# alphacep/vosk-tts

Hardware: AMD Instinct MI355X
Metric: audio_samples_per_sec (higher is better)
Workload: dtype f32

## Files before the change

### include/vits_mi355_debug.h

```cpp
#ifndef VITS_MI355_DEBUG_H
#define VITS_MI355_DEBUG_H
#include "vits_mi355.h"
#ifdef __cplusplus
extern "C" {
#endif

void vits_debug_force_tile(int mode);
void vits_debug_attention_impl(int impl);
void vits_debug_fast_path(int on);
void vits_debug_ks_waves(int nw);
void vits_debug_ln_stats(int on);
void vits_debug_persist(int mask);
void vits_debug_persist_spin(int limit);
void vits_debug_persist_when(int max_others_in_flight);
void vits_debug_persist_rearm_ms(int ms);
int vits_debug_persist_runs(vits_model* m);
void vits_debug_wn_fold(int on);
void vits_debug_conv_wp(int mode);
int vits_debug_decoder_needs(const vits_hparams* hp, int32_t* out, int32_t cap);
void vits_debug_conv_sp(int mode);
void vits_debug_no_bf16x3(int on);
void vits_debug_tail_impl(int impl);
void vits_debug_poison_workspace(int on);
int vits_debug_plain_attention(int device, const float* qkv, const int64_t* lengths, int32_t B, int32_t C, int32_t T,
                               int32_t n_heads, float* out);

int vits_debug_clock_probe(int device, int32_t duration_us, double* ghz, int32_t n);

#ifdef __cplusplus
}
#endif
#endif
```

### vosk_tts_amd/csrc/conv_small.hip.h

```cpp
#pragma once
#include "conv_mfma.hip.h"

#define C16_MAXU 20

template <typename F>
static void pack_conv_weights16(float* dst, int Mpad16, int Cin, int K, F src) {
  const int n_u = Cin / CONV_CI_T * K;
  for (int mb = 0; mb < Mpad16 / 16; ++mb)
    for (int u = 0; u < n_u; ++u)
      for (int lane = 0; lane < 64; ++lane)
        for (int q = 0; q < 4; ++q) {
          const int chunk = u / K, kk = u % K;
          const int ci = chunk * CONV_CI_T + 4 * q + (lane >> 4);
          const int row = mb * 16 + (lane & 15);
          dst[(((size_t)mb * n_u + u) * 64 + lane) * 4 + q] = src(row, ci, kk);
        }
}

static inline int c16_row_pitch(int row) { return row <= 16 ? 16 : (row <= 48 ? 48 : 80); }

#define DDS_MAXI 16
#define DDS_XP 36
__device__ __forceinline__ float c16_gelu(float v) { return 0.5f * v * (1.0f + erff(v * 0.70710678118654752440f)); }
template <int NG, int NC>
// ... 710 lines not shown
    return;
  }
  const bool masked = P.out_mask && ecol >= len_raw;
#pragma unroll
  for (int i = 0; i < NE; ++i) {
    float r = sum[i] + ebias[i];
    if (masked) r = 0.f;
    r += eres[i];
    if (eok[i]) {
      G.y[eoff[i]] = r;
      if (G.y2) G.y2[eoff[i]] = r;
    }
  }
  CONV_DBG(5);
}

template <int NW>
__global__ void __launch_bounds__(NW * 64, 4) conv_wp_kernel(const ConvParams P) {
  extern __shared__ float lds[];
  kernarg_warm<sizeof(ConvParams)>();
  const int tid = threadIdx.x, lane = tid & 63;
  const int wave = __builtin_amdgcn_readfirstlane(tid >> 6);
  CONV_DBG(0);
  int mt, grp, nt, b;
  if (!conv_decode_block(P, mt, grp, nt, b)) return;
  const ConvGroup& G = P.g[grp];
  switch (G.K) {
    case 3: conv_wp_body<NW, 3>(P, G, lds, mt, nt, b, wave, lane); break;
    case 7: conv_wp_body<NW, 7>(P, G, lds, mt, nt, b, wave, lane); break;
    case 11: conv_wp_body<NW, 11>(P, G, lds, mt, nt, b, wave, lane); break;
    default: conv_wp_body<NW, 0>(P, G, lds, mt, nt, b, wave, lane); break;
  }
}
```

### vosk_tts_amd/csrc/engine.hip

```cpp
#include <hip/hip_runtime.h>

#include <math.h>
#include <stdarg.h>
#include <stdio.h>
#include <stdlib.h>
#include <string.h>
#include <fcntl.h>
#include <sys/file.h>
#include <unistd.h>

#include <algorithm>
#include <atomic>
#include <chrono>
#include <map>
#include <mutex>
#include <string>
#include <tuple>
#include <vector>

#include "../../include/vits_mi355.h"
#include "../../include/vits_mi355_debug.h"
#include "conv_mfma.hip.h"
#include "conv_small.hip.h"
#include "conv_sp.hip.h"
#include "conv_bf3.hip.h"
#include "kernels_misc.hip.h"
#include "persist.hip.h"

static thread_local char g_err[512];
static int fail(int code, const char* fmt, ...) {
  va_list ap;
  va_start(ap, fmt);
  vsnprintf(g_err, sizeof g_err, fmt, ap);
  va_end(ap);
  return code;
}
#define HIP_TRY(expr)                                                                              \
  do {                                                                                             \
    hipError_t e_ = (expr);                                                                        \
    if (e_ != hipSuccess) return fail(VITS_ERR_DEVICE, "%s failed: %s (%s:%d)", #expr, hipGetErrorString(e_), __FILE__, __LINE__); \
  } while (0)
#define TRY(expr)              \
  do {                         \
    int rc_ = (expr);          \
// ... 467 lines not shown
  const long long until = g_ps_off_until_ns.load(), now = steady_ns();
  out->active_mask = (until && now < until) ? 0 : g_persist.load();
  out->off_for_ms = (until && now < until) ? (int32_t)((until - now + 999999) / 1000000) : 0;
  out->timeouts = g_ps_timeouts.load();
  out->rearms = g_ps_rearms.load();
  out->launches = -1;
  out->process_owns_device = -1;
  if (m) {
    out->launches = vits_debug_persist_runs(m);
    std::lock_guard<std::mutex> g(g_tok_mu);
    if (m->device >= 0 && m->device < 64) out->process_owns_device = g_proc_lock[m->device];
  }
  return VITS_OK;
}
void vits_debug_persist_spin(int limit) {
  const int lim = limit > 0 ? limit : 0;
  g_ps_spin_limit = lim;
  std::lock_guard<std::mutex> g(g_models_mu);
  for (vits_model* m : g_models) {
    hipSetDevice(m->device);
    hipDeviceSynchronize();
    hipMemcpy(m->ps_dbg, &lim, sizeof(int), hipMemcpyHostToDevice);
  }
}
int vits_debug_persist_runs(vits_model* m) {
  if (!m) return -1;
  int v[2] = {0, 0};
  hipSetDevice(m->device);
  hipDeviceSynchronize();
  if (hipMemcpy(v, m->ps_dbg, sizeof v, hipMemcpyDeviceToHost) != hipSuccess) return -1;
  return v[1];
}
void vits_debug_conv_wp(int mode) { g_wp_mode = mode; }
int vits_debug_decoder_needs(const vits_hparams* hp, int32_t* out, int32_t cap) {
  if (!hp || !out || hp->n_ups < 0 || hp->n_ups > VITS_MAX_UPS || hp->n_resd < 0 || hp->n_resd > VITS_MAX_RESD || hp->n_resk < 0 || hp->n_resk > VITS_MAX_RESK)
    return -fail(VITS_ERR_ARG, "decoder_needs: bad arguments");
  for (int i = 0; i < hp->n_ups; ++i) if (hp->up_rates[i] < 1) return -fail(VITS_ERR_ARG, "decoder_needs: bad up_rates");
  if (hp->dec_type < 0 || hp->dec_type > 3) return -fail(VITS_ERR_ARG, "decoder_needs: dec_type %d unsupported", hp->dec_type);
  if ((hp->dec_type == 0 || hp->dec_type == 2 || hp->dec_type == 3) && (hp->istft_hop < 1 || hp->subbands < 1 || hp->istft_n_fft < 1))
    return -fail(VITS_ERR_ARG, "decoder_needs: bad tail geometry");
  if ((hp->dec_type == 0 || hp->dec_type == 2) && hp->pqmf_taps < 0) return -fail(VITS_ERR_ARG, "decoder_needs: bad synthesis filter length");
  if (hp->dec_type == 3 && hp->subbands != 1) return -fail(VITS_ERR_ARG, "decoder_needs: single-band decoder with subbands != 1");
  const DecNeeds N = decoder_needs(*hp, true);
  std::vector<int32_t> v = {N.pre_out + 3, N.pre_out, N.post_out, N.tail_cols};
  for (int i = 0; i < hp->n_ups; ++i) {
    v.push_back(N.ups_q[i]);
    for (int d = 0; d < hp->n_resd; ++d) v.push_back(N.c1_out[i][d]);
    for (int d = 0; d < hp->n_resd; ++d) v.push_back(N.c2_out[i][d]);
  }
  for (int i = 0; i < (int)v.size() && i < cap; ++i) out[i] = v[i];
  return (int)v.size();
}
void vits_debug_conv_sp(int mode) { g_sp_mode = mode; }
int vits_debug_clock_probe(int device, int32_t duration_us, double* ghz, int32_t n) {
  if (!ghz || n < 1 || n > 1024 || duration_us < 1 || duration_us > 2000000 || device < 0 || device >= 64) return fail(VITS_ERR_ARG, "clock probe: bad arguments");
  HIP_TRY(hipSetDevice(device));
  static std::mutex mu;
  static hipStream_t st[64];
  static double* buf[64];
  std::lock_guard<std::mutex> g(mu);
  if (!st[device]) {
    HIP_TRY(hipStreamCreateWithFlags(&st[device], hipStreamNonBlocking));
    if (hipMalloc((void**)&buf[device], sizeof(double) * 1024) != hipSuccess) { buf[device] = nullptr; return fail(VITS_ERR_NOMEM, "clock probe: device alloc failed"); }
  }
  if (!buf[device]) return fail(VITS_ERR_NOMEM, "clock probe: no buffer");
  hipLaunchKernelGGL(clock_probe_kernel, dim3(n), dim3(64), 0, st[device], buf[device], (long long)duration_us * 100);
// ... 166 lines not shown
```

### vosk_tts_amd/csrc/engine_launch.hip.h

```cpp
#pragma once
struct ProfScope {
  vits_session* s; bool on;
  ProfScope(vits_session* s_, const char* name, double flops, const char* kernel = "-") : s(s_), on(s_->profile) {
    if (!on) return;
    ProfRec r; r.name = name; r.kernel = kernel; r.flops = flops;
    hipEventCreate(&r.e0); hipEventCreate(&r.e1);
    hipEventRecord(r.e0, s->stream);
    s->prof.push_back(r);
  }
  void set_kernel(const char* k) { if (on) s->prof.back().kernel = k; }
  void add_template_arg(int v) {
    if (!on) return;
    std::string& k = s->prof.back().kernel;
    if (!k.empty() && k.back() == '>') { k.pop_back(); k += "," + std::to_string(v) + ">"; }
  }
  ~ProfScope() { if (on) hipEventRecord(s->prof.back().e1, s->stream); }
};


static bool big_lds_needed(std::atomic<unsigned long long>& done);
static void persist_launch(vits_session* s, vits_session::PersistProg& pp, const char* name, const float* d_noise = nullptr, float nsw = 0.f,
                           uint64_t seed = 0, const int64_t* d_ids = nullptr, const int* d_forced = nullptr, float length_scale = 1.f,
                           float noise_scale = 0.f) {
  vits_model* m = s->m;
// ... 224 lines not shown
static thread_local int g_no_bf3 = 0;
static bool conv_wp_ok(const ConvParams& P, int epi, int halo, bool small) {
  static const int env_mode = getenv("VITS_CONV_WP") ? atoi(getenv("VITS_CONV_WP")) : 0;
  const int mode = g_wp_mode ? g_wp_mode : env_mode;
  if (mode == 1 || epi != EPI_STORE) return false;
  if (P.x_ch_sign != 1 || P.x_ch_off || P.tile_start || P.ups_u || P.reflect || P.in_scale != 1.f || P.ln_g || P.dds_y2 || P.ln_stat_out) return false;
  if (P.Cin % CONV_CI_T || P.Tin < 4 || 32 + halo > WP_PITCH || P.in_slope < 0.f || P.in_slope > 1.f) return false;
  if (P.x_split && (P.n_groups != 1 || P.x_split % CONV_CI_T || !P.g[0].x2)) return false;
  for (int g = 0; g < P.n_groups; ++g)
    if (P.g[g].x3 || (P.g[g].x2 && !P.x_split)) return false;
  if (mode == 2) return true;
  return small && P.Cin >= 8 * CONV_CI_T && (long)P.B * P.Tout >= 256;
}
static void launch_conv_wp(vits_session* s, ConvParams& P, ProfScope& ps) {
  constexpr int NW = 8;
  P.tile_start = nullptr;
  P.ntiles_m = cdiv(P.M, 32);
  P.ntiles_n = cdiv(P.Tout, 32);
  const size_t lds = (size_t)NW * CONV_CI_T * WP_PITCH * sizeof(float);
  int owned = 0;
  {
    const int per_xcd = cdiv(P.ntiles_m * P.ntiles_n, 8);
    if (P.B == 1 && P.n_groups == 3 && P.g[0].K >= P.g[1].K && P.g[1].K >= P.g[2].K && 3 * per_xcd <= 64 &&
        per_xcd <= 32) {
      P.xcd_mode = 11;
      owned = 8 * 3 * per_xcd;
    }
  }
  const dim3 grid(owned ? owned : P.ntiles_m * P.ntiles_n * P.B * P.n_groups);
  ps.set_kernel("conv_wp_kernel<8>");
  hipLaunchKernelGGL(conv_wp_kernel<NW>, grid, dim3(NW * 64), lds, s->stream, P);
}

static long c16_cols_conv(int epi) {
  return epi == EPI_GATE ? 512 : 256;
}
static constexpr long C16_COLS_DDS = 800;
static bool conv_takes_c16(const ConvParams& P, int epi) {
  const long c16_cols = c16_cols_conv(epi);
  if (!(g_force_tile == 3 || (g_force_tile == 0 && (long)P.B * P.Tout <= c16_cols))) return false;
  if (g_force_tile == 0 && (long)P.B * P.Tout > 192 && P.Cin >= 256 && !P.ln_g && !P.dds_y2 && !P.ln_stat_out &&
      conv_wp_ok(P, epi, (P.g[0].K - 1) * P.g[0].dil, true))
    return false;
  return c16_waves(P, epi) != 0;
}

static thread_local int g_sp_mode = -1;
static int sp_mode() { return g_sp_mode >= 0 ? g_sp_mode : 1; }
static bool conv_sp_ok(const ConvParams& P, int epi, int halo) {
  if (sp_mode() == 0 || epi == EPI_GATE) return false;
  if (P.Cin % SP_STAGE_CH || P.ups_u || P.reflect || P.x_split || P.ln_g || P.dds_y2 || P.ln_stat_out || 64 + halo > 128 || P.Tin < 2) return false;
  for (int g = 0; g < P.n_groups; ++g)
    if (P.g[g].x2 || P.g[g].x3) return false;
  return true;
}
template <int EPI>
static void launch_sp(vits_session* s, ConvParams& P, int halo) {
  attach_tile_table(s, P, 64);
  P.ntiles_m = cdiv(P.M, 64);
  P.ntiles_n = cdiv(P.Tout, 64);
  P.row_len = 64 + halo;
  const int nblk = P.ntiles_m * P.ntiles_n * P.B * P.n_groups;
  const size_t lds = (size_t)2 * 4 * P.row_len * SP_PITCH * sizeof(float);
  if (lds > 64 * 1024) {
    static std::atomic<unsigned long long> done1{0}, done2{0};
    if (P.row_len <= 64) { if (big_lds_needed(done1)) hipFuncSetAttribute((const void*)conv_sp_kernel<EPI, 1>, hipFuncAttributeMaxDynamicSharedMemorySize, 160 * 1024); }
// ... 89 lines not shown
    if (small) { ps.set_kernel("conv_mfma_ks_kernel<2,1,GATE,1>"); launch_ks<2, 1, EPI_GATE>(s, P, halo, &ps); }
    else if (!g_no_bf3 && P.g[0].wb && P.n_groups == 1 && P.M % 128 == 0 && P.x_ch_sign == 1 && !P.x_ch_off && !P.g[0].x2 && !P.ln_g &&
             P.in_scale >= 0.f && P.in_slope >= 0.f && P.in_slope <= 1.f &&
             (long)cdiv(P.M, 128) * cdiv(P.Tout, 128) * P.B >= 256) {
      ps.set_kernel("conv_bf3_kernel<2,GATE>");
      attach_tile_table(s, P, 128);
      P.ntiles_m = cdiv(P.M, 128);
      P.ntiles_n = cdiv(P.Tout, 128);
      P.row_len = 128 + halo;
      const size_t lds = (size_t)2 * 2 * P.row_len * (BF3_PITCH * 2);
      hipLaunchKernelGGL((conv_bf3_kernel<2, EPI_GATE>), dim3(P.ntiles_m * P.ntiles_n * P.B), dim3(256), lds, s->stream, P);
    } else {
      const long nblk64 = (long)cdiv(P.M, 128) * cdiv(P.Tout, 64) * P.B;
      if (g_force_tile == 0 && 32 + halo <= 64 && nblk64 >= 512 && nblk64 <= 1536) {
        ps.set_kernel("conv_mfma_kernel<2,1,2,1,GATE>"); launch_cfg<2, 1, 2, 1, EPI_GATE>(s, P, halo);
      } else {
        ps.set_kernel("conv_mfma_kernel<2,2,2,1,GATE>"); launch_cfg<2, 2, 2, 1, EPI_GATE>(s, P, halo);
      }
    }
    return;
  }
  if (epi == EPI_RESSKIP) {
    if (small) { ps.set_kernel("conv_mfma_ks_kernel<1,1,RESSKIP,1>"); launch_ks<1, 1, EPI_RESSKIP>(s, P, halo, &ps); }
    else if (g_force_tile == 0 && sp_takes(P, epi, halo)) { ps.set_kernel("conv_sp_kernel<RESSKIP>"); launch_sp<EPI_RESSKIP>(s, P, halo); }
    else { ps.set_kernel("conv_mfma_kernel<2,2,1,1,RESSKIP>"); launch_cfg<2, 2, 1, 1, EPI_RESSKIP>(s, P, halo); }
    return;
  }
  if (epi == EPI_COUPLE) {
    if (small) { ps.set_kernel("conv_mfma_ks_kernel<1,1,COUPLE,1>"); launch_ks<1, 1, EPI_COUPLE>(s, P, halo, &ps); }
    else if (g_force_tile == 0 && sp_takes(P, epi, halo)) { ps.set_kernel("conv_sp_kernel<COUPLE>"); launch_sp<EPI_COUPLE>(s, P, halo); }
    else { ps.set_kernel("conv_mfma_kernel<2,2,1,1,COUPLE>"); launch_cfg<2, 2, 1, 1, EPI_COUPLE>(s, P, halo); }
    return;
  }
  if (conv_wp_ok(P, epi, halo, small)) { launch_conv_wp(s, P, ps); return; }
  if (small) {
    const long blocks32 = (long)cdiv(P.M, 32) * cdiv(P.Tout, 32) * P.B * P.n_groups;
    const bool multi = P.g[0].x2 != nullptr;
    static const int ks_shape = getenv("VITS_KS_SHAPE") ? atoi(getenv("VITS_KS_SHAPE")) : 0;
    if (P.x_split) { ps.set_kernel("conv_mfma_ks_kernel<1,1,STORE,2>"); launch_ks<1, 1, EPI_STORE>(s, P, halo, &ps); return; }
    if (ks_shape == 12 || (ks_shape == 0 && blocks32 > 2048)) { ps.set_kernel(multi ? "conv_mfma_ks_kernel<1,2,STORE,3>" : "conv_mfma_ks_kernel<1,2,STORE,1>"); launch_ks<1, 2, EPI_STORE>(s, P, halo, &ps); }
    else { ps.set_kernel(multi ? "conv_mfma_ks_kernel<1,1,STORE,3>" : "conv_mfma_ks_kernel<1,1,STORE,1>"); launch_ks<1, 1, EPI_STORE>(s, P, halo, &ps); }
    return;
  }
  if ((P.ups_u && (P.ups_cout % 64)) || (!P.ups_u && P.M % 64 == 32)) {
    ps.set_kernel("conv_mfma_kernel<1,4,1,1,STORE>"); launch_cfg<1, 4, 1, 1, EPI_STORE>(s, P, halo); return;
  }
  auto bf3_ok = [&]() {
    bool ok = !g_no_bf3 && !P.reflect && !P.x_split && P.x_ch_sign == 1 && !P.x_ch_off && !P.ln_g;
    ok = ok && P.in_scale >= 0.f && P.in_slope >= 0.f && P.in_slope <= 1.f;
    if (P.ups_u && (P.ups_cout % 128 || P.n_groups != 1)) ok = false;
    for (int g = 0; g < P.n_groups; ++g) ok = ok && P.g[g].wb && !P.g[g].x2 && !P.g[g].x3;
    return ok;
  };
  auto bf3_go = [&](int mi) {
    ps.set_kernel(mi == 2 ? "conv_bf3_kernel<2>" : "conv_bf3_kernel<1>");
    attach_tile_table(s, P, 128);
    P.ntiles_m = cdiv(P.M, 64 * mi);
    P.ntiles_n = cdiv(P.Tout, 128);
    P.row_len = 128 + halo;
    const size_t lds = (size_t)2 * 2 * P.row_len * (BF3_PITCH * 2);
    const dim3 grid(P.ntiles_m * P.ntiles_n * P.B * P.n_groups);
    if (mi == 2) hipLaunchKernelGGL((conv_bf3_kernel<2, EPI_STORE>), grid, dim3(256), lds, s->stream, P);
    else hipLaunchKernelGGL((conv_bf3_kernel<1, EPI_STORE>), grid, dim3(256), lds, s->stream, P);
  };
  if (!P.ups_u && P.M == 64 && (long)cdiv(P.Tout, 128) * P.B * P.n_groups >= 512) {
    if (bf3_ok()) { bf3_go(1); return; }
    ps.set_kernel("conv_mfma_kernel<2,2,1,2,STORE>"); launch_cfg<2, 2, 1, 2, EPI_STORE>(s, P, halo); return;
// ... 120 lines not shown
```

### vosk_tts_amd/csrc/engine_session.hip.h

```cpp
#pragma once
struct ProfRec { std::string name; std::string kernel; hipEvent_t e0, e1; double flops; };

struct vits_session {
  vits_model* m = nullptr;
  hipStream_t stream = nullptr;
  bool own_stream = true;
  hipStream_t copy_stream = nullptr;
  char* arena = nullptr;
  size_t arena_bytes = 0, arena_used = 0;
  int* d_err = nullptr;
  int* h_err = nullptr;
  hipEvent_t ev0 = nullptr, ev1 = nullptr;
  bool timed = false;
  bool profile = false;
  std::vector<ProfRec> prof;
  typedef std::tuple<const void*, const void*, const void*, const void*, void*, int, int, int, uint64_t, float, float, float, int> GKey;
  std::map<GKey, hipGraphExec_t> graphs;
  bool use_graph = true;
  const SynthDev* dv = nullptr;
  const unsigned long long* item_seeds = nullptr;
  bool ragged = false;
  bool solo = false;

  int B = 0, Tx = 0, Ty = 0;
// ... 23 lines not shown
    double flops = 0;
  };
  PersistProg ps_enc, ps_sdp, ps_flow;
  PersistProg ps_front[2], ps_back, ps_full[2], ps_x;
  ll_t *ps_x_stats = nullptr, *ps_x_logw = nullptr, *ps_x_cum = nullptr, *ps_x_leny = nullptr, *ps_x_zp = nullptr;
  int ps_planned_roles = -1;
  int ps_roles = 7;
  bool ps_defer = false;
  PersistCtl* ps_ctl = nullptr;
  std::vector<std::pair<std::vector<long long>, const float*>> ps_pending;
  const float* ps_bert = nullptr;
  bool ps_owner = false;
  char* stage = nullptr;
  size_t stage_bytes = 0, stage_used = 0;

  int graph_nodes = 0;
  bool ea_pending = false;
  int ea_row = 0;
  bool rag_b1 = false;
  bool sdp_always = false;
  char *io_h = nullptr, *io_d = nullptr;
  size_t io_bytes = 0, io_len = 0, io_sid = 0, io_ids = 0, io_forced = 0, io_seeds = 0, io_bert = 0;
  int64_t* h_ylen = nullptr;
  hipGraphExec_t g1[8] = {nullptr, nullptr, nullptr, nullptr, nullptr, nullptr, nullptr, nullptr};
  std::map<int, vits_session*> backs;
  vits_session* front = nullptr;
  float* out_d = nullptr;
  int16_t* pcm_d = nullptr;
  char* out_h = nullptr;
  size_t out_elems = 0;
  hipGraphExec_t g2[8] = {nullptr, nullptr, nullptr, nullptr, nullptr, nullptr, nullptr, nullptr};
  uint64_t last_use = 0;
  size_t cache_bytes = 0;
};


template <typename T>
static T* bump(vits_session* s, size_t n) {
  size_t off = align_up(s->arena_used, 256);
  s->arena_used = off + n * sizeof(T);
  return s->arena ? reinterpret_cast<T*>(s->arena + off) : nullptr;
}

#include "persist_plan.hip.h"

static inline int persist_mask() { return tl_persist >= 0 ? tl_persist : 0; }
static int g_proc_lock[64];
static int g_proc_lock_fd[64];
static bool persist_process_lock(int dev) {
  if (g_proc_lock_fd[dev] == 0) {
    g_proc_lock_fd[dev] = -1;
    if (!(getenv("VITS_PERSIST_LOCK") && atoi(getenv("VITS_PERSIST_LOCK")) == 0)) {
      char bus[64] = "dev";
      if (hipDeviceGetPCIBusId(bus, (int)sizeof bus, dev) != hipSuccess) snprintf(bus, sizeof bus, "dev%d", dev);
      for (char* c = bus; *c; ++c) if (*c == ':' || *c == '.' || *c == '/') *c = '_';
      char path[512];
      snprintf(path, sizeof path, "%s/vits_mi355_persist_%s.lock", getenv("VITS_PERSIST_LOCK_DIR") ? getenv("VITS_PERSIST_LOCK_DIR") : "/tmp", bus);
      const int fd = open(path, O_CREAT | O_RDONLY | O_CLOEXEC | O_NOFOLLOW, 0644);
      if (fd > 0) g_proc_lock_fd[dev] = fd;
      else if (fd == 0) close(fd);
    }
  }
  if (g_proc_lock_fd[dev] < 0) { g_proc_lock[dev] = 1; return true; }
  if (flock(g_proc_lock_fd[dev], LOCK_EX | LOCK_NB) != 0) {
    if (g_proc_lock[dev] >= 0 && !getenv("VITS_QUIET"))
      fprintf(stderr, "[vits_mi355] device %d: another process is running the persistent programs: this call takes the launch path\n", dev);
// ... 89 lines not shown
    s->ps_x.ll = bump<ll_t>(s, s->ps_x.cells);
    ll_t* p = s->ps_x.ll;
    s->ps_x_stats = p; p += Tpx * 2 * I;
    s->ps_x_logw = p; p += Tpx;
    s->ps_x_cum = p; p += Tpx;
    s->ps_x_leny = p; p += 16;
    s->ps_x_zp = p;
  }
  s->zA = bump<float>(s, B * I * Ty); s->zB = bump<float>(s, B * I * Ty);
  s->fh = bump<float>(s, B * He * Ty); s->fx = bump<float>(s, B * H * Ty);
  s->facts = bump<float>(s, B * H * Ty * (size_t)(hp.flow_wn_layers > 0 ? hp.flow_wn_layers : 1));
  s->fskip = bump<float>(s, B * He * Ty);
  s->dec_bufs.clear();
  size_t C = hp.dec_initial_channel, T = Ty;
  s->dec_bufs.push_back(bump<float>(s, B * C * T));
  size_t stage_max = 0;
  {
    size_t c = C, t = T;
    for (int i = 0; i < hp.n_ups; ++i) { c /= 2; t *= hp.up_rates[i]; if (c * t > stage_max) stage_max = c * t; }
  }
  for (int k = 0; k < 14; ++k) s->dec_bufs.push_back(bump<float>(s, B * stage_max));
  if (hp.dec_type == 0 || hp.dec_type == 2 || hp.dec_type == 3) {
    size_t P = (size_t)hp.subbands * (hp.istft_n_fft + 2);
    size_t t = T; for (int i = 0; i < hp.n_ups; ++i) t *= hp.up_rates[i];
    s->dec_bufs.push_back(bump<float>(s, B * P * (t + 1)));
    s->dec_bufs.push_back(bump<float>(s, hp.dec_type == 3 ? 64 : B * hp.subbands * t * hp.istft_hop));
  } else {
    size_t t = T; for (int i = 0; i < hp.n_ups; ++i) t *= hp.up_rates[i];
    s->dec_bufs.push_back(bump<float>(s, B * t));
    s->dec_bufs.push_back(bump<float>(s, 64));
  }
}

static void drop_graphs(vits_session* s) {
  for (auto& kv : s->graphs) hipGraphExecDestroy(kv.second);
  s->graphs.clear();
}

static int session_reserve(vits_session* s, int B, int Tx, int Ty) {
  if (s->arena && B == s->B && Tx == s->Tx && Ty == s->Ty && s->ps_planned_roles == s->ps_roles) return VITS_OK;
  {
    const vits_hparams& hp = s->m->hp;
    int widest = hp.filter_channels;
    for (int c : {hp.dec_initial_channel, 2 * hp.hidden_channels, 2 * hp.inter_channels, hp.dp_filter_channels, hp.bert_dim})
      if (c > widest) widest = c;
    long long worst = (long long)widest * (Ty > Tx ? Ty : Tx);
    long long rate = 1;
    for (int i = 0; i < hp.n_ups && i < VITS_MAX_UPS; ++i) {
      rate *= hp.up_rates[i];
      const long long e = (long long)(hp.dec_initial_channel >> (i + 1)) * Ty * rate;
      if (e > worst) worst = e;
    }
    if (worst * 4 >= (1LL << 31)) return fail(VITS_ERR_ARG, "T_y = %d frames: a per-item decoder tensor would exceed 2 GiB", Ty);
  }
  drop_graphs(s);
  char* keep = s->arena;
  s->arena = nullptr;
  plan(s, B, Tx, Ty);
  const size_t need = s->arena_used + 4096;
  s->arena = keep;
  if (need > s->arena_bytes) {
    if (s->arena) { hipStreamSynchronize(s->stream); hipFree(s->arena); s->arena = nullptr; s->arena_bytes = 0; }
    const size_t want = need + need / 8;
    void* p = nullptr;
    if (hipMalloc(&p, want) != hipSuccess) { s->B = s->Tx = s->Ty = 0; return fail(VITS_ERR_NOMEM, "workspace hipMalloc of %zu bytes failed", want); }
    s->arena = static_cast<char*>(p);
    s->arena_bytes = want;
  }
  plan(s, B, Tx, Ty);
  s->ps_planned_roles = s->ps_roles;
  if (g_poison) {
    hipMemsetAsync(s->arena, 0xFF, s->arena_bytes, s->stream);
    hipStreamSynchronize(s->stream);
  }
  if (!s->ps_defer) persist_plan(s);
  return VITS_OK;
}

static int session_new(vits_model* m, vits_session** out) {
  vits_session* s = new vits_session();
  s->m = m;
  HIP_TRY(hipSetDevice(m->device));
  HIP_TRY(hipStreamCreateWithFlags(&s->stream, hipStreamNonBlocking));
  HIP_TRY(hipMalloc((void**)&s->d_err, sizeof(int)));
  HIP_TRY(hipMemsetAsync(s->d_err, 0, sizeof(int), s->stream));
  HIP_TRY(hipStreamSynchronize(s->stream));
  HIP_TRY(hipEventCreate(&s->ev0));
  HIP_TRY(hipEventCreate(&s->ev1));
  *out = s;
  return VITS_OK;
}

static void session_free(vits_session* s) {
  if (!s) return;
  hipSetDevice(s->m->device);
  if (s->stream) hipStreamSynchronize(s->stream);
  drop_graphs(s);
  for (auto& kv : s->backs) session_free(kv.second);
  s->backs.clear();
  for (int i = 0; i < 8; ++i) { if (s->g1[i]) hipGraphExecDestroy(s->g1[i]); if (s->g2[i]) hipGraphExecDestroy(s->g2[i]); }
  if (s->io_h) hipHostFree(s->io_h);
  if (s->io_d) hipFree(s->io_d);
  if (s->h_ylen) hipHostFree(s->h_ylen);
  if (s->out_d) hipFree(s->out_d);
  if (s->pcm_d) hipFree(s->pcm_d);
  if (s->out_h) hipHostFree(s->out_h);
  for (auto& r : s->prof) { hipEventDestroy(r.e0); hipEventDestroy(r.e1); }
  if (s->arena) hipFree(s->arena);
  if (s->ps_ctl) hipFree(s->ps_ctl);
  for (vits_session::PersistProg* pp : {&s->ps_enc, &s->ps_sdp, &s->ps_flow, &s->ps_front[0], &s->ps_front[1], &s->ps_back, &s->ps_full[0], &s->ps_full[1]}) {
    if (pp->d) hipFree(pp->d);
    if (pp->recs_d) hipFree(pp->recs_d);
  }
  if (s->stage) hipFree(s->stage);
  if (s->d_err) hipFree(s->d_err);
  if (s->h_err) hipHostFree(s->h_err);
  if (s->ev0) hipEventDestroy(s->ev0);
  if (s->ev1) hipEventDestroy(s->ev1);
  if (s->copy_stream) hipStreamDestroy(s->copy_stream);
  if (s->stream && s->own_stream) hipStreamDestroy(s->stream);
  delete s;
}

static int pool_acquire(vits_model* m, vits_session** out) {
  {
    std::lock_guard<std::mutex> g(m->pool_mu);
    if (!m->pool.empty()) { *out = m->pool.back(); m->pool.pop_back(); return VITS_OK; }
  }
  return session_new(m, out);
}
static void pool_release(vits_model* m, vits_session* s) {
  std::lock_guard<std::mutex> g(m->pool_mu);
  m->pool.push_back(s);
}
```

Measured before the change: 45.07 million.

## Add LPT-scheduled persistent conv kernel with split-K for decoder resblock convs

Adds a conv_wps kernel that runs a host-built longest-processing-time schedule of (group, m-tile, n-tile, channel-range) work items over two slots per CU. Optionally the largest-kernel group is split along input channels with partial-sum exchange through a global counter. The next item's weights, inputs and epilogue data are prefetched during the current item. The goal is to balance uneven per-group work (different kernel sizes) across CUs instead of using one block per tile. The cost is plan buffers cached per shape, atomics and syncs for split reduction, and a fallback to the old path when the plan is not multi-round.

```diff
diff --git a/include/vits_mi355_debug.h b/include/vits_mi355_debug.h
--- a/include/vits_mi355_debug.h
+++ b/include/vits_mi355_debug.h
@@ -17,6 +17,8 @@
 int vits_debug_persist_runs(vits_model* m);
 void vits_debug_wn_fold(int on);
 void vits_debug_conv_wp(int mode);
+void vits_debug_wp_sched(int mode);
+int vits_debug_wp_schedule(int32_t M, int32_t Cin, int32_t T, int32_t k0, int32_t k1, int32_t k2, int32_t n_cu, int32_t* out, int32_t cap);
 int vits_debug_decoder_needs(const vits_hparams* hp, int32_t* out, int32_t cap);
 void vits_debug_conv_sp(int mode);
 void vits_debug_no_bf16x3(int on);
diff --git a/vosk_tts_amd/csrc/conv_small.hip.h b/vosk_tts_amd/csrc/conv_small.hip.h
--- a/vosk_tts_amd/csrc/conv_small.hip.h
+++ b/vosk_tts_amd/csrc/conv_small.hip.h
@@ -766,3 +766,335 @@
     default: conv_wp_body<NW, 0>(P, G, lds, mt, nt, b, wave, lane); break;
   }
 }
+
+
+struct WpsArgs {
+  const int2* slots;
+  const int4* items;
+  float* part;
+  int* cnt;
+};
+struct WpsItem { int grp, mt, nt, c0, nch, split; };
+__device__ __forceinline__ WpsItem wps_item(const WpsArgs& S, int i) {
+  const int4 q = S.items[i];
+  WpsItem it;
+  it.grp = __builtin_amdgcn_readfirstlane(q.x & 15);
+  it.mt = __builtin_amdgcn_readfirstlane(q.x >> 4);
+  it.nt = __builtin_amdgcn_readfirstlane(q.y);
+  it.c0 = __builtin_amdgcn_readfirstlane(q.z & 0xffff);
+  it.nch = __builtin_amdgcn_readfirstlane(q.z >> 16);
+  it.split = __builtin_amdgcn_readfirstlane(q.w);
+  return it;
+}
+template <int NW>
+struct WpsPre {
+  f32x4 a[2][2];
+  f32x4 v0[4], v1[4];
+  float ebias[16 / NW], eres[16 / NW];
+};
+template <int NW>
+__device__ __forceinline__ void wps_prefetch(const ConvParams& P, const WpsItem& it, int wave, int lane, WpsPre<NW>& pre) {
+  constexpr int NE = 16 / NW;
+  const ConvGroup& G = P.g[it.grp];
+  const int K = G.K, dil = G.dil;
+  const int n0 = it.nt * 32, m0 = it.mt * 32;
+  int mb = m0 >> 5;
+  if (mb >= (P.M >> 5)) mb = 0;
+  const f32x4* wp = reinterpret_cast<const f32x4*>(G.w) + (size_t)mb * G.n_sg * 64 + lane;
+  const size_t sg = 2 * (size_t)(it.c0 + wave) * K;
+  pre.a[0][0] = wp[sg * 64];
+  pre.a[0][1] = wp[(sg + 1) * 64];
+  pre.a[1][0] = wp[(sg + 2) * 64];
+  pre.a[1][1] = wp[(sg + 3) * 64];
+  const int nvec = (32 + (K - 1) * dil + 3) >> 2;
+  const int t_base = n0 - G.pad_l;
+  const int r4 = lane >> 4, v16 = lane & 15;
+  const unsigned lrow = (unsigned)(r4 * P.Tin_stride);
+  const float* xc = G.x + (long long)(it.c0 + wave) * CONV_CI_T * P.Tin_stride;
+#pragma unroll
+  for (int ps = 0; ps < 2; ++ps) {
+    if (ps == 1 && nvec <= 16) break;
+    const int tv = t_base + 4 * (v16 + 16 * ps);
+    const int tc0 = tv < 0 ? 0 : tv;
+    const int tc = tc0 > P.Tin - 4 ? P.Tin - 4 : tc0;
+    f32x4 (&v)[4] = ps ? pre.v1 : pre.v0;
+#pragma unroll
+    for (int j = 0; j < 4; ++j)
+      v[j] = *reinterpret_cast<const f32x4u*>(reinterpret_cast<const char*>(xc + 4 * j * P.Tin_stride) + (lrow + (unsigned)tc) * 4u);
+  }
+  const int h = lane >> 5, ecol = n0 + (lane & 31);
+  const int ecolc = ecol < P.Tout ? ecol : P.Tout - 1;
+#pragma unroll
+  for (int i = 0; i < NE; ++i) {
+    const int e = NE * wave + i;
+    const int r = m0 + 4 * h + (e & 3) + 8 * (e >> 2);
+    const int rc = r < P.Cout ? r : P.Cout - 1;
+    const float bv = (G.bias ? G.bias : G.w)[rc];
+    const float rv = (G.res ? G.res : G.y)[(long long)rc * P.Tout_stride + ecolc];
+    pre.ebias[i] = G.bias ? bv : 0.f;
+    pre.eres[i] = G.res ? rv : 0.f;
+  }
+}
+
+template <int NW, int KT>
+__device__ __forceinline__ void wps_body(const ConvParams& P, const WpsArgs& S, float* lds, const WpsItem& it, const WpsItem& nx, bool has_next,
+                                         WpsPre<NW>& pre, int len_raw, int t_lim_in, int wave, int lane) {
+  constexpr int NE = 16 / NW;
+  const int tid = threadIdx.x;
+  const ConvGroup& G = P.g[it.grp];
+  const int h = lane >> 5, l31 = lane & 31;
+  const int n0 = it.nt * 32, m0 = it.mt * 32;
+  const int K = KT ? KT : G.K, dil = G.dil;
+  const int c_first = it.c0 + wave;
+  const int my_chunks = (it.nch - wave + NW - 1) / NW;
+  const int last_c = c_first + NW * (my_chunks - 1);
+  float ebias[NE], eres[NE];
+#pragma unroll
+  for (int i = 0; i < NE; ++i) { ebias[i] = pre.ebias[i]; eres[i] = pre.eres[i]; }
+  int mb = m0 >> 5;
+  if (mb >= (P.M >> 5)) mb = 0;
+  const f32x4* wp = reinterpret_cast<const f32x4*>(G.w) + (size_t)mb * G.n_sg * 64 + lane;
+  f32x4 (&a)[2][2] = pre.a;
+  int lci = K > 2 ? 0 : 1, lk = K > 2 ? 2 : 0;
+  auto load_a_half = [&](f32x4 (&d)[2], int half) {
+    const int c = c_first + NW * lci;
+    const bool live = c <= last_c;
+    const size_t sg = 2 * ((size_t)(live ? c : last_c) * K + (live ? lk : K - 1));
+    d[half] = wp[(sg + half) * 64];
+    if (half) {
+      ++lk;
+      if (lk == K) { lk = 0; ++lci; }
+    }
+  };
+  auto load_a = [&](f32x4 (&d)[2]) { load_a_half(d, 0); load_a_half(d, 1); };
+  const int row_len = 32 + (K - 1) * dil;
+  const int nvec = (row_len + 3) >> 2;
+  const bool two = nvec > 16;
+  const int t_base = n0 - G.pad_l;
+  const int r4 = lane >> 4, v16 = lane & 15;
+  int tvp[2], tcp[2];
+#pragma unroll
+  for (int ps = 0; ps < 2; ++ps) {
+    tvp[ps] = t_base + 4 * (v16 + 16 * ps);
+    const int tc = tvp[ps] < 0 ? 0 : tvp[ps];
+    tcp[ps] = tc > P.Tin - 4 ? P.Tin - 4 : tc;
+  }
+  const unsigned lrow = (unsigned)(r4 * P.Tin_stride);
+  float* sl = lds + wave * (CONV_CI_T * WP_PITCH);
+  float* sw = sl + r4 * WP_PITCH + 4 * v16;
+  const float slope = P.in_slope;
+  f32x4 (&v0)[4] = pre.v0;
+  f32x4 (&v1)[4] = pre.v1;
+  auto load_slab = [&](int ci) {
+    const float* xc = G.x + (long long)(c_first + NW * ci) * CONV_CI_T * P.Tin_stride;
+#pragma unroll
+    for (int j = 0; j < 4; ++j)
+      v0[j] = *reinterpret_cast<const f32x4u*>(reinterpret_cast<const char*>(xc + 4 * j * P.Tin_stride) + (lrow + (unsigned)tcp[0]) * 4u);
+    if (two) {
+#pragma unroll
+      for (int j = 0; j < 4; ++j)
+        v1[j] = *reinterpret_cast<const f32x4u*>(reinterpret_cast<const char*>(xc + 4 * j * P.Tin_stride) + (lrow + (unsigned)tcp[1]) * 4u);
+    }
+  };
+  const int ecol = n0 + l31;
+  const int t_lim = t_lim_in;
+  const bool interior = t_base >= 0 && t_base + 4 * nvec <= t_lim;
+  auto put = [&](f32x4 (&v)[4], int ps) {
+    if (v16 + 16 * ps >= nvec) return;
+    if (interior && slope == 1.f) {
+#pragma unroll
+      for (int j = 0; j < 4; ++j) *reinterpret_cast<f32x4*>(sw + 4 * j * WP_PITCH + 64 * ps) = v[j];
+    } else if (interior) {
+#pragma unroll
+      for (int j = 0; j < 4; ++j) {
+        f32x4 o;
+#pragma unroll
+        for (int q = 0; q < 4; ++q) o[q] = fmaxf(v[j][q], v[j][q] * slope);
+        *reinterpret_cast<f32x4*>(sw + 4 * j * WP_PITCH + 64 * ps) = o;
+      }
+    } else {
+      const int sh = tvp[ps] - tcp[ps];
+#pragma unroll
+      for (int j = 0; j < 4; ++j) {
+        f32x4 o;
+#pragma unroll
+        for (int q = 0; q < 4; ++q) {
+          const int t = tvp[ps] + q, idx = q + sh;
+          const float x = idx <= 0 ? v[j][0] : (idx == 1 ? v[j][1] : (idx == 2 ? v[j][2] : v[j][3]));
+          o[q] = (t >= 0 && t < t_lim) ? fmaxf(x, x * slope) : 0.f;
+        }
+        *reinterpret_cast<f32x4*>(sw + 4 * j * WP_PITCH + 64 * ps) = o;
+      }
+    }
+  };
+  auto stage = [&]() {
+    put(v0, 0);
+    if (two) put(v1, 1);
+  };
+  f32x16 acc;
+#pragma unroll
+  for (int e = 0; e < 16; ++e) acc[e] = 0.f;
+  const float* bl = sl + h * WP_PITCH + l31;
+  auto read_b = [&](float (&d)[8], int tap) {
+#pragma unroll
+    for (int p = 0; p < 8; ++p) d[p] = bl[2 * p * WP_PITCH + tap * dil];
+  };
+  auto mfma8 = [&](const f32x4 (&w)[2], const float (&d)[8]) {
+#pragma unroll
+    for (int p = 0; p < 8; ++p) acc = __builtin_amdgcn_mfma_f32_32x32x2f32(w[p >> 2][p & 3], d[p], acc, 0, 0, 0);
+  };
+  auto taps = [&](auto par) {
+    constexpr int PAR = decltype(par)::value;
+    float bb[2][8];
+    read_b(bb[0], 0);
+    if (KT) {
+#pragma unroll
+      for (int tap = 0; tap < (KT ? KT : 1); ++tap) {
+        f32x4 (&w)[2] = a[(tap + PAR) & 1];
+        const float (&d)[8] = bb[tap & 1];
+        if (tap + 1 < KT) read_b(bb[(tap + 1) & 1], tap + 1);
+        __builtin_amdgcn_sched_barrier(0);
+#pragma unroll
+        for (int p = 0; p < 4; ++p) acc = __builtin_amdgcn_mfma_f32_32x32x2f32(w[0][p], d[p], acc, 0, 0, 0);
+        load_a_half(w, 0);
+#pragma unroll
+        for (int p = 4; p < 8; ++p) acc = __builtin_amdgcn_mfma_f32_32x32x2f32(w[1][p & 3], d[p], acc, 0, 0, 0);
+        load_a_half(w, 1);
+        __builtin_amdgcn_sched_barrier(0);
+      }
+    } else {
+#pragma unroll 1
+      for (int tap = 0; tap < K; tap += 2) {
+        read_b(bb[1], tap + 1 < K ? tap + 1 : tap);
+        mfma8(a[PAR], bb[0]);
+        load_a(a[PAR]);
+        if (tap + 1 < K) {
+          read_b(bb[0], tap + 2 < K ? tap + 2 : tap + 1);
+          mfma8(a[PAR ^ 1], bb[1]);
+          load_a(a[PAR ^ 1]);
+        }
+      }
+    }
+  };
+  auto swap_slots = [&]() {
+    const f32x4 t0 = a[0][0], t1 = a[0][1];
+    a[0][0] = a[1][0]; a[0][1] = a[1][1];
+    a[1][0] = t0; a[1][1] = t1;
+  };
+  constexpr bool FLIP = KT & 1;
+#pragma unroll 1
+  for (int ci = 0; ci < my_chunks; ci += 2) {
+    stage();
+    if (ci + 1 < my_chunks) load_slab(ci + 1);
+    taps(wp_int<0>{});
+    if (!KT && (K & 1)) swap_slots();
+    if (ci + 1 < my_chunks) {
+      stage();
+      if (ci + 2 < my_chunks) load_slab(ci + 2);
+      taps(wp_int<FLIP ? 1 : 0>{});
+      if (!KT && (K & 1)) swap_slots();
+    }
+  }
+  if (has_next) wps_prefetch<NW>(P, nx, wave, lane, pre);
+  __builtin_amdgcn_sched_barrier(0);
+#pragma unroll
+  for (int e = 0; e < 16; ++e) sl[e * 64 + lane] = acc[e];
+  __syncthreads();
+  float sum[NE];
+#pragma unroll
+  for (int ee = 0; ee < NE; ++ee) {
+    float r = 0.f;
+#pragma unroll
+    for (int w = 0; w < NW; ++w) r += lds[w * (CONV_CI_T * WP_PITCH) + (NE * wave + ee) * 64 + lane];
+    sum[ee] = r;
+  }
+  if (has_next) __syncthreads();
+  if (it.split >= 0) {
+    const int half = it.c0 != 0;
+    float* mine = S.part + ((size_t)it.split * 2 + half) * 1024;
+    const float* other = S.part + ((size_t)it.split * 2 + (half ^ 1)) * 1024;
+#pragma unroll
+    for (int i = 0; i < NE; ++i) mine[(NE * wave + i) * 64 + lane] = sum[i];
+    asm volatile("s_waitcnt vmcnt(0)" ::: "memory");
+    __syncthreads();
+    int* flag = reinterpret_cast<int*>(lds + NW * CONV_CI_T * WP_PITCH);
+    if (tid == 0) {
+      __builtin_amdgcn_fence(__ATOMIC_RELEASE, "agent");
+      asm volatile("s_waitcnt vmcnt(0)" ::: "memory");
+      const int old = __hip_atomic_fetch_add(S.cnt + it.split, 1, __ATOMIC_RELAXED, __HIP_MEMORY_SCOPE_AGENT);
+      if (old == 1) {
+        __builtin_amdgcn_fence(__ATOMIC_ACQUIRE, "agent");
+        asm volatile("s_waitcnt vmcnt(0)" ::: "memory");
+        __hip_atomic_store(S.cnt + it.split, 0, __ATOMIC_RELAXED, __HIP_MEMORY_SCOPE_AGENT);
+      }
+      *flag = old;
+    }
+    __syncthreads();
+    const int last = __builtin_amdgcn_readfirstlane(*flag);
+    if (last != 1) return;
+#pragma unroll
+    for (int i = 0; i < NE; ++i) {
+      const float o = other[(NE * wave + i) * 64 + lane];
+      sum[i] = half ? o + sum[i] : sum[i] + o;
+    }
+  }
+  const bool masked = P.out_mask && ecol >= len_raw;
+#pragma unroll
+  for (int i = 0; i < NE; ++i) {
+    const int e = NE * wave + i;
+    const int r = m0 + 4 * h + (e & 3) + 8 * (e >> 2);
+    float v = sum[i] + ebias[i];
+    if (masked) v = 0.f;
+    v += eres[i];
+    if (ecol < P.Tout && r < P.Cout) {
+      const long long o = (long long)r * P.Tout_stride + ecol;
+      G.y[o] = v;
+      if (G.y2) G.y2[o] = v;
+    }
+  }
+}
+
+template <int NW>
+__global__ void __launch_bounds__(NW * 64, 4) conv_wps_kernel(const ConvParams P, const WpsArgs S) {
+  extern __shared__ float lds[];
+  kernarg_warm<sizeof(ConvParams) + sizeof(WpsArgs)>();
+  const int lane = threadIdx.x & 63;
+  const int wave = __builtin_amdgcn_readfirstlane(threadIdx.x >> 6);
+  const int2 rg = S.slots[blockIdx.x];
+  const int i0 = __builtin_amdgcn_readfirstlane(rg.x), end = i0 + __builtin_amdgcn_readfirstlane(rg.y);
+  int len_raw = 0x7fffffff, rag_raw = 0x7fffffff, rag_cap = 0x7fffffff;
+  if (P.in_mask || P.out_mask || P.skip_len) len_raw = __builtin_amdgcn_readfirstlane(P.len[0]);
+  if (P.rag) { rag_raw = __builtin_amdgcn_readfirstlane(P.rag[0]); rag_cap = __builtin_amdgcn_readfirstlane(P.rag[1]); }
+  int n_lim = 0x7fffffff, t_lim = P.Tin;
+  if (P.skip_len) n_lim = len_raw;
+  if (P.in_mask) t_lim = len_raw < t_lim ? len_raw : t_lim;
+  if (P.rag) {
+    const int ol = conv_rag_limit(rag_raw, rag_cap, P.rag_out_mul, P.rag_out_add, P.rag_out_cap_add);
+    n_lim = ol < n_lim ? ol : n_lim;
+    const int il = conv_rag_limit(rag_raw, rag_cap, P.rag_in_mul, P.rag_in_add);
+    t_lim = il < t_lim ? il : t_lim;
+  }
+  auto next_live = [&](int i) {
+    while (i < end && __builtin_amdgcn_readfirstlane(S.items[i].y) * 32 >= n_lim) ++i;
+    return i;
+  };
+  int i = next_live(i0);
+  if (i >= end) return;
+  WpsItem it = wps_item(S, i);
+  WpsPre<NW> pre;
+  wps_prefetch<NW>(P, it, wave, lane, pre);
+  for (;;) {
+    const int j = next_live(i + 1);
+    const bool has_next = j < end;
+    const WpsItem nx = has_next ? wps_item(S, j) : it;
+    switch (P.g[it.grp].K) {
+      case 3: wps_body<NW, 3>(P, S, lds, it, nx, has_next, pre, len_raw, t_lim, wave, lane); break;
+      case 7: wps_body<NW, 7>(P, S, lds, it, nx, has_next, pre, len_raw, t_lim, wave, lane); break;
+      case 11: wps_body<NW, 11>(P, S, lds, it, nx, has_next, pre, len_raw, t_lim, wave, lane); break;
+      default: wps_body<NW, 0>(P, S, lds, it, nx, has_next, pre, len_raw, t_lim, wave, lane); break;
+    }
+    if (!has_next) break;
+    i = j;
+    it = nx;
+  }
+}
diff --git a/vosk_tts_amd/csrc/engine.hip b/vosk_tts_amd/csrc/engine.hip
--- a/vosk_tts_amd/csrc/engine.hip
+++ b/vosk_tts_amd/csrc/engine.hip
@@ -10,6 +10,7 @@
 #include <unistd.h>
 
 #include <algorithm>
+#include <array>
 #include <atomic>
 #include <chrono>
 #include <map>
@@ -543,6 +544,20 @@
   return v[1];
 }
 void vits_debug_conv_wp(int mode) { g_wp_mode = mode; }
+void vits_debug_wp_sched(int mode) { g_wps_mode = mode; }
+int vits_debug_wp_schedule(int32_t M, int32_t Cin, int32_t T, int32_t k0, int32_t k1, int32_t k2, int32_t n_cu, int32_t* out, int32_t cap) {
+  if (M < 32 || M % 32 || Cin < 16 || Cin % CONV_CI_T || T < 1 || n_cu < 1 || n_cu > 4096 || k0 < 2 || k1 < 2 || k2 < 2 || !out)
+    return -fail(VITS_ERR_ARG, "wp_schedule: bad arguments");
+  const int K[3] = {k0, k1, k2};
+  const WpsPlan pl = wps_build(M, Cin, T, K, n_cu);
+  std::vector<int32_t> v{(int32_t)pl.slots.size(), (int32_t)pl.items.size(), pl.n_split, pl.use ? 1 : 0, (int32_t)pl.max_cu, (int32_t)pl.sum};
+  for (const int2& q : pl.slots) { v.push_back(q.x); v.push_back(q.y); }
+  for (const int4& q : pl.items) {
+    v.push_back(q.x & 15); v.push_back(q.x >> 4); v.push_back(q.y); v.push_back(q.z & 0xffff); v.push_back(q.z >> 16); v.push_back(q.w);
+  }
+  for (size_t i = 0; i < v.size() && i < (size_t)cap; ++i) out[i] = v[i];
+  return (int)v.size();
+}
 int vits_debug_decoder_needs(const vits_hparams* hp, int32_t* out, int32_t cap) {
   if (!hp || !out || hp->n_ups < 0 || hp->n_ups > VITS_MAX_UPS || hp->n_resd < 0 || hp->n_resd > VITS_MAX_RESD || hp->n_resk < 0 || hp->n_resk > VITS_MAX_RESK)
     return -fail(VITS_ERR_ARG, "decoder_needs: bad arguments");
diff --git a/vosk_tts_amd/csrc/engine_launch.hip.h b/vosk_tts_amd/csrc/engine_launch.hip.h
--- a/vosk_tts_amd/csrc/engine_launch.hip.h
+++ b/vosk_tts_amd/csrc/engine_launch.hip.h
@@ -280,6 +280,123 @@
   hipLaunchKernelGGL(conv_wp_kernel<NW>, grid, dim3(NW * 64), lds, s->stream, P);
 }
 
+static thread_local int g_wps_mode = 0;
+struct WpsPlan {
+  std::vector<int2> slots;
+  std::vector<int4> items;
+  int n_split = 0;
+  long max_cu = 0, sum = 0;
+  bool use = false;
+};
+static WpsPlan wps_lpt(int ntm, int ntn, int nch, const int (&K)[3], int n_cu, bool split) {
+  struct It { long w; int grp, mt, nt, c0, nch, split; };
+  std::vector<It> v;
+  int n_split = 0;
+  for (int g = 0; g < 3; ++g)
+    for (int nt = 0; nt < ntn; ++nt)
+      for (int mt = 0; mt < ntm; ++mt) {
+        if (split && g == 0) {
+          v.push_back({(long)K[g] * (nch / 2), g, mt, nt, 0, nch / 2, n_split});
+          v.push_back({(long)K[g] * (nch - nch / 2), g, mt, nt, nch / 2, nch - nch / 2, n_split});
+          ++n_split;
+        } else {
+          v.push_back({(long)K[g] * nch, g, mt, nt, 0, nch, -1});
+        }
+      }
+  std::stable_sort(v.begin(), v.end(), [](const It& a, const It& b) { return a.w > b.w; });
+  std::vector<long> cu_load(n_cu, 0), slot_load(2 * n_cu, 0);
+  std::vector<std::vector<int>> per_slot(2 * n_cu);
+  WpsPlan pl;
+  for (int i = 0; i < (int)v.size(); ++i) {
+    int c = 0;
+    for (int k = 1; k < n_cu; ++k) if (cu_load[k] < cu_load[c]) c = k;
+    cu_load[c] += v[i].w;
+    const int sl = slot_load[c + n_cu] < slot_load[c] ? c + n_cu : c;
+    slot_load[sl] += v[i].w;
+    per_slot[sl].push_back(i);
+    pl.sum += v[i].w;
+  }
+  for (long l : cu_load) pl.max_cu = l > pl.max_cu ? l : pl.max_cu;
+  for (int sl = 0; sl < 2 * n_cu; ++sl) {
+    pl.slots.push_back(make_int2((int)pl.items.size(), (int)per_slot[sl].size()));
+    for (int i : per_slot[sl]) {
+      const It& t = v[i];
+      pl.items.push_back(make_int4(t.grp | t.mt << 4, t.nt, t.c0 | t.nch << 16, t.split));
+    }
+  }
+  pl.n_split = n_split;
+  return pl;
+}
+static WpsPlan wps_build(int M, int Cin, int T, const int (&K)[3], int n_cu) {
+  constexpr int NW = 8;
+  const int ntm = M / 32, ntn = cdiv(T, 32), nch = Cin / CONV_CI_T;
+  WpsPlan pl = wps_lpt(ntm, ntn, nch, K, n_cu, false);
+  const bool multi_round = (long)3 * ntm * ntn > 2L * n_cu;
+  pl.use = multi_round;
+  if (nch >= 2 * NW) {
+    WpsPlan sp = wps_lpt(ntm, ntn, nch, K, n_cu, true);
+    if (sp.max_cu < pl.max_cu) { sp.use = true; return sp; }
+  }
+  return pl;
+}
+static vits_session::WpsDev* wps_get(vits_session* s, int M, int Cin, int T, const int (&K)[3]) {
+  const int n_cu = s->m->n_cu;
+  const std::array<int, 7> key{M, Cin, T, K[0], K[1], K[2], n_cu};
+  auto it = s->wps.find(key);
+  if (it != s->wps.end()) return &it->second;
+  hipStreamCaptureStatus cs = hipStreamCaptureStatusNone;
+  if (hipStreamIsCapturing(s->stream, &cs) != hipSuccess || cs != hipStreamCaptureStatusNone) return nullptr;
+  const WpsPlan pl = wps_build(M, Cin, T, K, n_cu);
+  const size_t b_slots = pl.slots.size() * sizeof(int2), b_items = pl.items.size() * sizeof(int4);
+  const size_t o_items = align_up(b_slots, 256), o_cnt = align_up(o_items + b_items, 256), o_part = align_up(o_cnt + (size_t)pl.n_split * 4, 256);
+  const size_t bytes = o_part + (size_t)pl.n_split * 2 * 1024 * sizeof(float);
+  vits_session::WpsDev d;
+  if (hipMalloc((void**)&d.buf, bytes) != hipSuccess) { (void)hipGetLastError(); return nullptr; }
+  hipMemcpy(d.buf, pl.slots.data(), b_slots, hipMemcpyHostToDevice);
+  hipMemcpy(d.buf + o_items, pl.items.data(), b_items, hipMemcpyHostToDevice);
+  if (pl.n_split) hipMemset(d.buf + o_cnt, 0, (size_t)pl.n_split * 4);
+  d.n_slots = (int)pl.slots.size();
+  d.use = pl.use;
+  d.slots = reinterpret_cast<int2*>(d.buf);
+  d.items = reinterpret_cast<int4*>(d.buf + o_items);
+  d.cnt = reinterpret_cast<int*>(d.buf + o_cnt);
+  d.part = reinterpret_cast<float*>(d.buf + o_part);
+  return &(s->wps[key] = d);
+}
+static void wps_prepare_decoder(vits_session* s) {
+  vits_model* m = s->m;
+  const vits_hparams& hp = m->hp;
+  if (s->B != 1 || hp.n_resk != 3 || m->n_cu < 8 || g_wps_mode == 1 || m->rb.empty()) return;
+  long T = s->Ty;
+  for (int i = 0; i < hp.n_ups; ++i) {
+    T *= hp.up_rates[i];
+    int K[3];
+    for (int j = 0; j < 3; ++j) K[j] = m->rb[(size_t)i * 3 + j].K;
+    std::sort(K, K + 3, [](int a, int b) { return a > b; });
+    if (T > 0 && T < (1 << 26)) wps_get(s, m->rb[(size_t)i * 3].c1[0].Mpad, m->ups[i].cout, (int)T, K);
+  }
+}
+static bool launch_conv_wps(vits_session* s, ConvParams& P, ProfScope& ps) {
+  constexpr int NW = 8;
+  if (g_wps_mode == 1 || s->m->n_cu < 8) return false;
+  if (P.B != 1 || P.n_groups != 3 || P.x_split || P.bias_b || P.scale_b || P.relu || P.M % 32 || P.Cin % CONV_CI_T || P.Cin / CONV_CI_T < NW ||
+      P.Cin / CONV_CI_T > 0xffff || P.Tin < 4)
+    return false;
+  int K[3];
+  for (int g = 0; g < 3; ++g) {
+    if (P.g[g].K < 2 || !P.g[g].x || P.g[g].x2 || P.g[g].x3) return false;
+    K[g] = P.g[g].K;
+  }
+  vits_session::WpsDev* d = wps_get(s, P.M, P.Cin, P.Tout, K);
+  if (!d || !(d->use || g_wps_mode == 2)) return false;
+  P.tile_start = nullptr;
+  WpsArgs S{d->slots, d->items, d->part, d->cnt};
+  const size_t lds = (size_t)NW * CONV_CI_T * WP_PITCH * sizeof(float) + 16;
+  ps.set_kernel("conv_wps_kernel<8>");
+  hipLaunchKernelGGL(conv_wps_kernel<NW>, dim3(d->n_slots), dim3(NW * 64), lds, s->stream, P, S);
+  return true;
+}
+
 static long c16_cols_conv(int epi) {
   return epi == EPI_GATE ? 512 : 256;
 }
@@ -435,7 +552,10 @@
     else { ps.set_kernel("conv_mfma_kernel<2,2,1,1,COUPLE>"); launch_cfg<2, 2, 1, 1, EPI_COUPLE>(s, P, halo); }
     return;
   }
-  if (conv_wp_ok(P, epi, halo, small)) { launch_conv_wp(s, P, ps); return; }
+  if (conv_wp_ok(P, epi, halo, small)) {
+    if (!launch_conv_wps(s, P, ps)) launch_conv_wp(s, P, ps);
+    return;
+  }
   if (small) {
     const long blocks32 = (long)cdiv(P.M, 32) * cdiv(P.Tout, 32) * P.B * P.n_groups;
     const bool multi = P.g[0].x2 != nullptr;
diff --git a/vosk_tts_amd/csrc/engine_session.hip.h b/vosk_tts_amd/csrc/engine_session.hip.h
--- a/vosk_tts_amd/csrc/engine_session.hip.h
+++ b/vosk_tts_amd/csrc/engine_session.hip.h
@@ -79,6 +79,8 @@
   hipGraphExec_t g2[8] = {nullptr, nullptr, nullptr, nullptr, nullptr, nullptr, nullptr, nullptr};
   uint64_t last_use = 0;
   size_t cache_bytes = 0;
+  struct WpsDev { char* buf = nullptr; int n_slots = 0; bool use = false; int2* slots = nullptr; int4* items = nullptr; float* part = nullptr; int* cnt = nullptr; };
+  std::map<std::array<int, 7>, WpsDev> wps;
 };
 
 
@@ -234,6 +236,8 @@
   }
 }
 
+static void wps_prepare_decoder(vits_session* s);
+
 static void drop_graphs(vits_session* s) {
   for (auto& kv : s->graphs) hipGraphExecDestroy(kv.second);
   s->graphs.clear();
@@ -275,6 +279,7 @@
     hipMemsetAsync(s->arena, 0xFF, s->arena_bytes, s->stream);
     hipStreamSynchronize(s->stream);
   }
+  wps_prepare_decoder(s);
   if (!s->ps_defer) persist_plan(s);
   return VITS_OK;
 }
@@ -315,6 +320,7 @@
     if (pp->recs_d) hipFree(pp->recs_d);
   }
   if (s->stage) hipFree(s->stage);
+  for (auto& kv : s->wps) if (kv.second.buf) hipFree(kv.second.buf);
   if (s->d_err) hipFree(s->d_err);
   if (s->h_err) hipHostFree(s->h_err);
   if (s->ev0) hipEventDestroy(s->ev0);
```

Result: slower. 37.76 million (median of 2 runs) (-16.2%).
